# Kkuntal990/video-to-video-diffusion

Measured on AMD Instinct MI355X. Metric: ddim_steps_per_sec, higher is better.
Workload: dtype bf16; 1 GPU; DDIM-50 step (U-Net eval + update) on latent [1, 8, 48, 128, 128] = 8->48 slices @512x512, effective 264.66M U-Net (128x(1,2,4,4), latent 8), one volume per GPU, hipGraph-captured step; volumes_per_gpu=1, parallelism=dp1, full=False, finite_outputs=True

## Files before the change

### include/ctsi.h

```cpp
#ifndef CTSI_H
#define CTSI_H

#include <stddef.h>
#include <stdint.h>

#ifdef __cplusplus
extern "C" {
#endif

#define CTSI_OK 0
#define CTSI_ERR_INVALID (-1)
#define CTSI_ERR_UNSUPPORTED (-2)
#define CTSI_ERR_HIP (-3)

int ctsi_version(void);
int ctsi_ablation_build(void);
const char* ctsi_last_error(void);
int ctsi_device_available(void);

int ctsi_ncdhw_f32_to_ndhwc_bf16(const float* src, void* dst, int n, int c, int d, int h, int w,
                                 int c_total, int c_off, void* stream);
int ctsi_ndhwc_bf16_to_ncdhw_f32(const void* src, float* dst, int n, int c, int d, int h, int w,
                                 void* stream);
int ctsi_ncdhw_f32_to_ndhwc_f32(const float* src, float* dst, int n, int c, int d, int h, int w,
// ... 26 lines not shown
    const double* gn_sums;
    const float* gn_gamma;
    const float* gn_beta;
    int gn_groups;
    float gn_eps;
    long long gn_count;
    int gn_silu;
    void* workspace;
} ctsi_conv_out;

int ctsi_conv_plan_create(ctsi_conv_plan** plan, const ctsi_conv_desc* desc);
int ctsi_conv_plan_set_weight_cin(ctsi_conv_plan* plan, int cin_w);
int ctsi_conv_plan_set_stream_tail(ctsi_conv_plan* plan, int on);
void ctsi_conv_plan_destroy(ctsi_conv_plan* plan);
int ctsi_conv_plan_out_dims(const ctsi_conv_plan* plan, int* d_out, int* h_out, int* w_out);
size_t ctsi_conv_plan_weight_bytes(const ctsi_conv_plan* plan);
int ctsi_conv_plan_tiles(const ctsi_conv_plan* plan);
int ctsi_conv_plan_tiles_per_sample(const ctsi_conv_plan* plan);
int ctsi_conv_plan_cout_pad(const ctsi_conv_plan* plan);
size_t ctsi_conv_plan_workspace_bytes(const ctsi_conv_plan* plan);
double ctsi_conv_plan_flops(const ctsi_conv_plan* plan);
int ctsi_conv_plan_config(const ctsi_conv_plan* plan, int* bm, int* bn, int* mode);
int ctsi_conv_plan_form(const ctsi_conv_plan* plan, int out[8]);
#define CTSI_PACK_GATHER 1
#define CTSI_PACK_GATHER_SMALL 2
#define CTSI_PACK_HALO 3
#define CTSI_PACK_K32 4
#define CTSI_PACK_HEAD 5
#define CTSI_PACK_STREAM_TAIL 6
#define CTSI_PACK_STEM 7
int ctsi_conv_plan_pack_layout(const ctsi_conv_plan* plan);
int ctsi_conv_plan_pack_weights(const ctsi_conv_plan* plan, const float* w_f32, void* packed,
                                void* stream);
int ctsi_conv_fwd(const ctsi_conv_plan* plan, const void* x1, const void* x2, const void* packed_w,
                  const float* bias, const ctsi_conv_out* out, void* stream);

int ctsi_gn_colsum(const void* x_bf16, float* colsum, int n, int c, int d, int h, int w,
                   int* tiles_per_sample, void* stream);
int ctsi_gn_colsum_tiles(int d, int h, int w);
int ctsi_gn_finalize(const float* colsum, double* sums, int n, int c, int c_pad, int groups,
                     int tiles_per_sample, int nclass, int accumulate, void* stream);
int ctsi_gn_apply(const void* x_bf16, void* y_bf16, const double* sums, const float* gamma,
                  const float* beta, int n, int c, int d, int h, int w, int d_stat, int groups, float eps,
                  int silu_pre, const float* tbias, int tbias_stride, const int* step_ptr,
                  const void* residual_bf16, int silu_post, void* stream);

// ... 201 lines not shown
```

### video-to-video-diffusion_amd/csrc/conv3_halo_k32.hip

```cpp
#include "conv3_halo_common.h"
#include <stdlib.h>
#include <type_traits>

template <int NJ, bool DIRECT>
__device__ __forceinline__ int hk_col(int j, int r16) { return DIRECT ? r16 * NJ + j : j * 16 + r16; }

template <int TD_, int TH_, int TW_ = 32, int BN_ = 128, int UPS_ = 2>
struct HkCfg {
    static constexpr int TD = TD_, TH = TH_, TW = TW_, UPS = UPS_;
    static constexpr int HD = TD + 2, HH = TH + 2, HW = TW + 2;
    static constexpr int HV = HD * HH * HW;
    static constexpr int HALO_INSTR = (HV + 31) / 32;
    static constexpr int HALO_BYTES = HALO_INSTR * 1024;
    static constexpr int BM = TD * TH * TW;
    static constexpr int BN = BN_;
    static constexpr int NJ = BN / 16;
    static constexpr int TAP_BYTES = BN * 32;
    static constexpr int STEP_TAPS = 2 * UPS;
    static constexpr int WSLOT_BYTES = STEP_TAPS * TAP_BYTES;
    static constexpr int NWS = 4;
    static constexpr int NWAVE = 8;
    static constexpr int MA = BM / 128;
    static constexpr int NTH = 64 * NWAVE;
    static constexpr int NPIECE = (HALO_INSTR + NWAVE - 1) / NWAVE;
// ... 35 lines not shown
#if defined(__HIP_DEVICE_COMPILE__)
    using Cfg = HkCfg<TD_, TH_, TW_, BN_, UPS_>;
    constexpr int UPS = Cfg::UPS, NJ = Cfg::NJ, NJH = Cfg::NJ / 2, STEP_TAPS = Cfg::STEP_TAPS;
    constexpr int TAPS = (TR || DS) ? 12 : 27;
    static_assert(!(TR && DS), "one form at a time");
    constexpr int MA = Cfg::MA;
    constexpr int TH = Cfg::TH, TW = Cfg::TW, HH = Cfg::HH, HW = Cfg::HW, HV = Cfg::HV;
    constexpr int HALO_INSTR = Cfg::HALO_INSTR, HALO_BYTES = Cfg::HALO_BYTES, BM = Cfg::BM, BN = Cfg::BN;
    constexpr int TAP_BYTES = Cfg::TAP_BYTES, WSLOT_BYTES = Cfg::WSLOT_BYTES, NWS = Cfg::NWS, NWAVE = Cfg::NWAVE;
    constexpr int NTH = Cfg::NTH, NPIECE = Cfg::NPIECE, OFF_W = Cfg::OFF_W, OFF_ROW = Cfg::OFF_ROW, OFF_CS = Cfg::OFF_CS;
    constexpr int BNP = Cfg::BNP;
    extern __shared__ __attribute__((aligned(16))) char smem[];
    long long* s_rowoff = reinterpret_cast<long long*>(smem + OFF_ROW);
    float* s_cs = reinterpret_cast<float*>(smem + OFF_CS);

    const int tid = threadIdx.x;
    const int lane = tid & 63;
    const int wave = __builtin_amdgcn_readfirstlane(tid >> 6);

    HK_STAMP(0);
    if ((CTSI_DBG(p.dbg, 4096)) && tid == 0 && blockIdx.x < HK_NSTAMP)
        g_hk_stamps[blockIdx.x][7] = ((unsigned long long)__builtin_amdgcn_s_getreg((31 << 11) | (0 << 6) | 20) << 32) |
                                     (unsigned)__builtin_amdgcn_s_getreg((31 << 11) | (0 << 6) | 4);
    int bid = xcd_remap_h(blockIdx.x, gridDim.x);
    const int khalf = SK ? (bid & 1) : 0;
    if (SK) bid >>= 1;
    int mt, nt, cls = 0;
    if (TR) {
        const int ns = 4 * p.ntiles_n;
        const int G = (p.n_major > 0 && p.n_major < ns && ns % p.n_major == 0) ? p.n_major : ns;
        const int per_g = p.mtiles * G;
        const int sg = bid / per_g;
        const int rem = bid - sg * per_g;
        mt = rem / G;
        const int sib = sg * G + (rem - mt * G);
        cls = sib / p.ntiles_n;
        nt = sib - cls * p.ntiles_n;
    } else {
        h3_decode_tile(bid, p.mtiles, p.ntiles_n, p.n_major, &mt, &nt);
    }
    const int py = cls >> 1, px = cls & 1;
    const int n0 = nt * BN;
    const int nchunks = SK ? p.nchunks / 2 : p.nchunks;
    const int cbase = khalf * nchunks;
    const int nb = mt / p.tps;
    int r0 = mt - nb * p.tps;
    int tD, tH, tW;
    if (p.tile_order == 1) {
        tH = r0 / (p.tilesD * p.tilesW);
        r0 -= tH * p.tilesD * p.tilesW;
        tD = r0 / p.tilesW;
        tW = r0 - tD * p.tilesW;
    } else if (p.tile_order == 2 && (p.tilesW & 3) == 0 && (p.tilesH & 7) == 0) {
        tD = r0 / (p.tilesH * p.tilesW);
        r0 -= tD * p.tilesH * p.tilesW;
        const int st = r0 >> 5, in = r0 & 31, spr = p.tilesW >> 2;
        tW = (st % spr) * 4 + (in & 3);
        tH = (st / spr) * 8 + (in >> 2);
    } else {
        tD = r0 / (p.tilesH * p.tilesW);
        r0 -= tD * p.tilesH * p.tilesW;
        tH = r0 / p.tilesW;
        tW = r0 - tH * p.tilesW;
    }
    const int d0 = tD * Cfg::TD, h0 = tH * TH, w0 = tW * TW;

// ... 227 lines not shown
                hfree = ((TAPS * hc - 1) >> 1) / UPS;
                ++hc;
            }
        }
        if (s + NWS - 1 < S && !(CTSI_DBG(p.dbg, 2))) {
            issue_weights(s + NWS - 1);
            n_w = 2;
        }
        n_prev = urgent ? n_w : n_w + n_halo;
        __builtin_amdgcn_sched_barrier(0);
    };
#define HK_UNIT(FAc, FAn, BADDR, UU, BADDR_N, UU_N, AADDR_N, MID)                                              \
    {                                                                                                          \
        if (!(CTSI_DBG(p.dbg, 128))) HK_LOAD_B(fbh, NJH, BADDR, UU);    \
        HK_LOAD_A(FAn, 0, AADDR_N);                                                                            \
        HK_MFMA(FAc, fbl, 0);                                                                                  \
        HK_SCHED();                                                                                            \
        MID;                                                                                                   \
        HK_LOAD_A(FAn, 2, AADDR_N);                                                                            \
        HK_LOAD_B(fbl, 0, BADDR_N, UU_N);                                                                      \
        HK_MFMA(FAc, fbh, NJH);                                                                                \
        HK_SCHED();                                                                                            \
    }
    for (int s = 0; s < S; ++s) {
        const int baddr = b_lane + (s % NWS) * WSLOT_BYTES;
        const int baddr_n = b_lane + ((s + 1) % NWS) * WSLOT_BYTES;
        const int q0 = STEP_TAPS * s;
        int an[UPS];
#pragma unroll
        for (int k = 0; k < UPS; ++k) {
            const int oa = tap_off(q0 + 2 * k + 2), ob = tap_off(q0 + 2 * k + 3);
            an[k] = a_lane + (tap1 ? ob : oa);
        }
        HK_UNIT(fa0, fa1, baddr, 0, baddr, 1, an[0], );
        if constexpr (UPS == 4) {
            HK_UNIT(fa1, fa0, baddr, 1, baddr, 2, an[1], );
            HK_UNIT(fa0, fa1, baddr, 2, baddr, 3, an[2], );
        }
        hk_wait_vm(n_prev);
        if (!(CTSI_DBG(p.dbg, 64))) __builtin_amdgcn_s_barrier();
        __builtin_amdgcn_sched_barrier(0);
        HK_UNIT(fa1, fa0, baddr, UPS - 1, baddr_n, 0, an[UPS - 1], if (wave < 4 || (CTSI_DBG(p.dbg, 16))) issue_group(s));
        if (wave >= 4 && !(CTSI_DBG(p.dbg, 16))) issue_group(s);
    }
#undef HK_UNIT
#undef HK_LOAD_A
#undef HK_LOAD_B
#undef HK_MFMA
#undef HK_SCHED
    HK_STAMP(2);
    asm volatile("s_waitcnt vmcnt(0) lgkmcnt(0)" ::: "memory");
    if (!(DIRECT && !SK) || (p.dbg_epi_barrier != 0)) __syncthreads();
    HK_STAMP(3);

    if (CTSI_DBG(p.dbg, 8)) return;
    if (SK) {
        const int tile = mt * p.ntiles_n + nt;
        constexpr int NREG = MA * NJ * 4;
        float* wsl = p.sk_ws + (size_t)tile * NREG * NTH + tid;
        int* s_role = reinterpret_cast<int*>(s_cs);
        if (tid == 0) {
            const int tk = __hip_atomic_fetch_add(p.sk_sync + 2 * tile, 1, __ATOMIC_RELAXED, __HIP_MEMORY_SCOPE_AGENT);
            if (tk >= 2) {
                atomicAdd(&g_hk_device_error[0], 1u);
                g_hk_device_error[1] = (unsigned)tile;
            }
            *s_role = tk & 1;
        }
        __syncthreads();
        const int role = *s_role;
        __syncthreads();
        if (role == 0) {
#pragma unroll
            for (int i = 0; i < MA; ++i)
#pragma unroll
                for (int j = 0; j < NJ; ++j)
#pragma unroll
                    for (int q = 0; q < 4; ++q)
                        __hip_atomic_store(wsl + (size_t)((i * NJ + j) * 4 + q) * NTH, acc[i][j][q], __ATOMIC_RELAXED,
                                           __HIP_MEMORY_SCOPE_AGENT);
            asm volatile("s_waitcnt vmcnt(0)" ::: "memory");
            __syncthreads();
            if (tid == 0) __hip_atomic_store(p.sk_sync + 2 * tile + 1, 1, __ATOMIC_RELAXED, __HIP_MEMORY_SCOPE_AGENT);
            return;
        }
        if (tid == 0) {
            int spins = 0;
            while (__hip_atomic_load(p.sk_sync + 2 * tile + 1, __ATOMIC_RELAXED, __HIP_MEMORY_SCOPE_AGENT) == 0 && spins < (1 << 22)) {
                __builtin_amdgcn_s_sleep(4);
                ++spins;
            }
            if (spins >= (1 << 22)) {
                atomicAdd(&g_hk_device_error[0], 1u);
                g_hk_device_error[1] = (unsigned)tile;
            } else {
                __hip_atomic_store(p.sk_sync + 2 * tile, 0, __ATOMIC_RELAXED, __HIP_MEMORY_SCOPE_AGENT);
                __hip_atomic_store(p.sk_sync + 2 * tile + 1, 0, __ATOMIC_RELAXED, __HIP_MEMORY_SCOPE_AGENT);
            }
        }
        __syncthreads();
#pragma unroll
        for (int i = 0; i < MA; ++i)
#pragma unroll
            for (int j = 0; j < NJ; ++j)
#pragma unroll
                for (int q = 0; q < 4; ++q)
                    acc[i][j][q] += __hip_atomic_load(wsl + (size_t)((i * NJ + j) * 4 + q) * NTH, __ATOMIC_RELAXED,
                                                      __HIP_MEMORY_SCOPE_AGENT);
    }
    bf16_t* s_tile = reinterpret_cast<bf16_t*>(smem);
    const bool want_sums = p.colsum != nullptr;
    unsigned vbits = 0;
#pragma unroll
    for (int i = 0; i < MA; ++i)
#pragma unroll
        for (int q = 0; q < 4; ++q)
            vbits |= (unsigned)(s_rowoff[wave * 16 * MA + 16 * i + (VPERM ? 4 * q + kg : 4 * kg + q)] >= 0) << (4 * i + q);
    auto tile_out = [&](auto masked_tag, auto sums_tag) {
        constexpr bool MASKED = decltype(masked_tag)::value, SUMS = decltype(sums_tag)::value;
#pragma unroll
        for (int j = 0; j < NJ; ++j) {
            const int col = hk_col<NJ, DIRECT>(j, r16);
            float s1 = 0.0f, s2 = 0.0f;
// ... 196 lines not shown
    return CTSI_OK;
}

extern "C" int ctsi_conv3_halo_k32_direct(int tile, int ksplit, int ds) {
#ifdef HK_STAGED_EPILOGUE
    return 0;
#else
    const bool t512 = tile == 0 || tile == 2, narrow = tile == 6 || tile == 7;
    return (t512 || narrow || (tile == 5 && ksplit == 2 && !ds)) ? 1 : 0;
#endif
}

template <int TD, int TH, int TW, int BN, int UPS, bool TR, bool SK = false, bool DS = false>
static void hk_launch(const Conv3HaloParams* hp, hipStream_t stream) {
    using Cfg = HkCfg<TD, TH, TW, BN, UPS>;
#ifdef HK_STAGED_EPILOGUE
    constexpr bool DIRECT = false;
#else
    constexpr bool DIRECT = TD * TH * TW == 512 || TW == 24 || TW == 12 || (SK && !DS);
#endif
    auto k = conv3_halo_k32_kernel<TD, TH, TW, BN, UPS, TR, SK, DS, DIRECT>;
    static CtsiPerDeviceOnce attr_once;
    if (attr_once.first()) hipFuncSetAttribute((const void*)k, hipFuncAttributeMaxDynamicSharedMemorySize, 160 * 1024);
    hipLaunchKernelGGL(k, dim3((TR ? 4 : 1) * (SK ? 2 : 1) * hp->mtiles * hp->ntiles_n), dim3(Cfg::NTH), Cfg::LDS_BYTES, stream,
                       *hp);
}

extern "C" size_t ctsi_conv3_halo_k32_splitk_bytes(int tiles) {
    const size_t sync = ((size_t)tiles * 8 + 255) / 256 * 256;
    return sync + (size_t)tiles * (4 * 8 * 4) * 512 * sizeof(float);
}

extern "C" int ctsi_conv3_halo_k32_launch(const Conv3HaloParams* hp, int tile ,
                                          int bn, void* stream) {
    CTSI_CHECK_ARG(bn == 128 && (tile == 0 || tile == 2 || tile == 3 || tile == 5 || tile == 6 || tile == 7),
                   "ctsi_conv3_halo_k32_launch: bad BN %d / tile %d", bn, tile);
    if (tile == 6 || tile == 7) {
        CTSI_CHECK_ARG(!(hp->ds && hp->tr) && !(hp->ksplit == 2 && (hp->ds || hp->tr)),
                       "ctsi_conv3_halo_k32_launch: tile %d has no split-K form for strided / transposed layers", tile);
        if (hp->ksplit == 2) {
            CTSI_CHECK_ARG(hp->sk_ws && hp->sk_sync && hp->nchunks % 8 == 0, "ctsi_conv3_halo_k32_launch: split-K needs its workspace");
            if (tile == 6)
                hk_launch<4, 4, 24, 128, 2, false, true>(hp, (hipStream_t)stream);
            else
                hk_launch<8, 4, 12, 128, 2, false, true>(hp, (hipStream_t)stream);
        } else if (hp->ds) {
            CTSI_CHECK_ARG(hp->Hi == 2 * hp->Ho && hp->Wi == 2 * hp->Wo && hp->C2 == 0 && hp->nchunks % 4 == 0,
                           "ctsi_conv3_halo_k32_launch: the Downsample form needs even input planes and one source");
            if (tile == 6)
                hk_launch<4, 4, 24, 128, 2, false, false, true>(hp, (hipStream_t)stream);
            else
                hk_launch<8, 4, 12, 128, 2, false, false, true>(hp, (hipStream_t)stream);
        } else if (hp->tr) {
            if (tile == 6)
                hk_launch<4, 4, 24, 128, 2, true>(hp, (hipStream_t)stream);
            else
                hk_launch<8, 4, 12, 128, 2, true>(hp, (hipStream_t)stream);
        } else if (tile == 6) {
            hk_launch<4, 4, 24, 128, 2, false>(hp, (hipStream_t)stream);
// ... 70 lines not shown
```

### video-to-video-diffusion_amd/csrc/conv_mfma.hip

```cpp
#include <type_traits>
#include "conv3_halo_common.h"
#include "conv_plan.h"
#include <string.h>
#include <stdlib.h>
#include <math.h>


__device__ __attribute__((aligned(256))) uint32_t g_ctsi_zero_page[64];

struct ConvKParams {
    const bf16_t* x1;
    const bf16_t* x2;
    const bf16_t* w;
    const float* bias;
    void* y;
    float* colsum;
    int C1, C2, Cin;
    int Di, Hi, Wi;
    int Dr, Hr, Wr;
    int sH, sW;
    int lTH, lTW;
    int linear;
    int tilesD, tilesH, tilesW, tps, mtiles;
    int ntiles_n;
// ... 797 lines not shown
            if (p->d.transposed && !nm) h.n_major = 4;
        }
        {
            h.dbg = ctsi_debug_flags();
            h.nchunks = ctsi_debug_ksteps(h.nchunks);
        }
        {
            const char* to = getenv("CTSI_CONV_TILE_ORDER");
            h.tile_order = to ? atoi(to) : 2;
            const char* eb = getenv("CTSI_CONV_EPI_BARRIER");
            h.dbg_epi_barrier = eb ? atoi(eb) : 0;
        }
        if (family == CONV_HEAD) {
            if (p->head2 && o->colsum == nullptr)
                return ctsi_conv3_head2_launch(&h, p->d.n, (const char*)packed_w + head1_bytes(p), o->mode, o->act, o->sn, o->sc, o->sd,
                                               o->sh, o->sw, stream);
            return ctsi_conv3_head_launch(&h, p->d.cout <= 8 ? 8 : 16, o->mode, o->act, o->sn, o->sc, o->sd, o->sh, o->sw, stream);
        }
        h.tr = p->d.transposed;
        if (family == CONV_K32 && p->ksplit == 2) {
            CTSI_CHECK_ARG(o->workspace, "ctsi_conv_fwd: this plan needs ctsi_conv_out.workspace (ctsi_conv_plan_workspace_bytes)");
            const int tiles = p->mtiles * p->ntiles_n;
            h.ksplit = 2;
            h.sk_sync = (int*)o->workspace;
            h.sk_ws = (float*)((char*)o->workspace + ((size_t)tiles * 8 + 255) / 256 * 256);
        }
        if (family == CONV_K32) return ctsi_conv3_halo_k32_launch(&h, p->form->code, p->BN, stream);
        return ctsi_conv3_halo_launch(&h, p->form->code, stream);
    }
    CTSI_CHECK_ARG(!p->form, "ctsi_conv_fwd: the 3x3x3 halo-tile plan supports bf16 NDHWC output without activation");
    ConvKParams k;
    memset(&k, 0, sizeof(k));
    k.x1 = (const bf16_t*)x1;
    k.x2 = (const bf16_t*)(x2 ? x2 : x1);
    k.w = (const bf16_t*)packed_w;
    k.bias = bias;
    k.y = o->y;
    k.colsum = o->colsum;
    k.C1 = p->d.c1; k.C2 = p->d.c2; k.Cin = p->Cin;
    k.Di = p->d.di; k.Hi = p->d.hi; k.Wi = p->d.wi;
    k.Dr = p->Dr; k.Hr = p->Hr; k.Wr = p->Wr;
    k.sH = p->sH; k.sW = p->sW;
    k.lTH = p->lTH; k.lTW = p->lTW;
    k.linear = p->linear;
    k.tilesD = p->tilesD; k.tilesH = p->tilesH; k.tilesW = p->tilesW; k.tps = p->tps; k.mtiles = p->mtiles;
    k.ntiles_n = p->ntiles_n;
// ... 46 lines not shown
```

### video-to-video-diffusion_amd/csrc/conv_plan.h

```cpp
#pragma once
#include "ctsi_internal.h"

#define CTSI_MAX_TAPS 48
#define CTSI_BK 64

enum ConvFamily {
    CONV_GATHER,
    CONV_HALO32,
    CONV_K32,
    CONV_HEAD,
};

struct ConvForm {
    ConvFamily family;
    int mode;
    int td, th, tw;
    int bn;
    int code;
    double eff;
    const char* name;
};

struct ctsi_conv_plan {
    ctsi_conv_desc d;
    int Cin, CinW;
    int Do, Ho, Wo;
    int Dr, Hr, Wr, sH, sW, uH, uW;
    int nclass, T;
    int small, lcpt, kc_per_tap, ksteps, Ktot;
    int BM, BN, CoutPad, ntiles_n;
    int lTH, lTW, TD, TH, TW, tilesD, tilesH, tilesW, tps, mtiles;
    int linear;
    int tapk[CTSI_MAX_TAPS];
    int tapdelta[CTSI_MAX_TAPS];
    int8_t od[CTSI_MAX_TAPS], oh[CTSI_MAX_TAPS], ow[CTSI_MAX_TAPS];
    int NA, NB, NC;
    int ad[4][4], bh[4][4], cw[4][4];
    int8_t pH[4], pW[4];
    int tap_margin[4], ad_min[4];
    int fast, dshift;
    const ConvForm* form;
    int gsplit;
    int ds;
    int head2;
    int ksplit;
    int stem;
    int stream1;
    double flops;
};

static inline ConvFamily conv_family(const ctsi_conv_plan* p) { return p->form ? p->form->family : CONV_GATHER; }
static inline int conv_k32_image(const ctsi_conv_plan* p) { return p->ds ? 2 : p->d.transposed; }
static inline int conv_k32_direct(const ctsi_conv_plan* p) { return ctsi_conv3_halo_k32_direct(p->form->code, p->ksplit, p->ds); }
static inline size_t head1_bytes(const ctsi_conv_plan* p) {
    return ((size_t)p->Cin * 27 * (p->d.cout <= 8 ? 8 : 16) * 2 + 1024 + 255) / 256 * 256;
}
```

### video-to-video-diffusion_amd/csrc/conv_plan.hip

```cpp
#include "conv_plan.h"
#include <string.h>
#include <stdlib.h>

static const double EFF_HALO32 = 1.0, EFF_HALO32_192 = 0.95, EFF_K32_512 = 1.15, EFF_K32_384 = 1.1, EFF_K32_NARROW = 1.07;
static const double EFF_PICK_W16 = 0.85, EFF_PICK_512 = 1.1, EFF_PICK_512_W16 = 1.0;
static const double EFF_ST_512 = 1.0, EFF_ST_384 = 0.96;
static const double EFF_GATHER_STANDIN = 0.6;

enum FormId { H32_4x2x32, H32_4x4x16, H32_3x4x16, K32_4x4x32, K32_4x8x16, K32_3x4x32, K32_3x8x16, K32_4x4x24, K32_8x4x12, HEAD_4x2x16,
              N_FORMS };
static const ConvForm FORMS[N_FORMS] = {
    {CONV_HALO32, 4, 4, 2, 32, 128, 1, EFF_HALO32, "halo32 4x2x32"},
    {CONV_HALO32, 4, 4, 4, 16, 128, 3, EFF_HALO32, "halo32 4x4x16"},
    {CONV_HALO32, 4, 3, 4, 16, 128, 4, EFF_HALO32_192, "halo32 3x4x16"},
    {CONV_K32, 9, 4, 4, 32, 128, 0, EFF_K32_512, "k32 4x4x32"},
    {CONV_K32, 9, 4, 8, 16, 128, 2, EFF_K32_512, "k32 4x8x16"},
    {CONV_K32, 9, 3, 4, 32, 128, 3, EFF_K32_384, "k32 3x4x32"},
    {CONV_K32, 9, 3, 8, 16, 128, 5, EFF_K32_384, "k32 3x8x16"},
    {CONV_K32, 9, 4, 4, 24, 128, 6, EFF_K32_NARROW, "k32 4x4x24"},
    {CONV_K32, 9, 8, 4, 12, 128, 7, EFF_K32_NARROW, "k32 8x4x12"},
    {CONV_HEAD, 8, 4, 2, 16, 16, 0, 1.0, "head 4x2x16"},
};
static int form_voxels(const ConvForm& f) { return f.td * f.th * f.tw; }
static const ConvForm* k32_sized(const ConvForm* f, bool v384) {
    return &FORMS[f->tw == 16 ? (v384 ? K32_3x8x16 : K32_4x8x16) : (v384 ? K32_3x4x32 : K32_4x4x32)];
}

enum Tri { UNSET = -1, OFF = 0, ON = 1 };
enum SplitK { SK_UNSET, SK_OFF, SK_ON, SK_PLAIN, SK_512 };
struct PlanEnv {
    bool no_halo3, force_halo3, no_c16, no_head3, no_head2, no_fast;
    Tri m512, m512w16, k32_384, k32t, k32d, narrow, narrow_sk, linear;
    int halo_tile;
    int h32w16;
    SplitK splitk;
    int sk384_min, sk512_min;
    bool has_gsplit; int gsplit;
    int tile_bm, tile_bn;
};
static Tri env_tri(const char* name) {
    const char* e = getenv(name);
    return e && !strcmp(e, "0") ? OFF : e && !strcmp(e, "1") ? ON : UNSET;
}
static int env_int(const char* name, int unset) {
    const char* e = getenv(name);
    return e ? atoi(e) : unset;
}
static PlanEnv read_plan_env() {
    PlanEnv e;
    e.no_halo3 = getenv("CTSI_CONV_NO_HALO3") != nullptr;
    e.force_halo3 = getenv("CTSI_CONV_FORCE_HALO3") != nullptr;
    e.no_c16 = getenv("CTSI_CONV_NO_C16") != nullptr;
    e.no_head3 = getenv("CTSI_CONV_NO_HEAD3") != nullptr;
    e.no_head2 = getenv("CTSI_CONV_NO_HEAD2") != nullptr;
    e.no_fast = getenv("CTSI_CONV_NO_FAST") != nullptr;
    e.m512 = env_tri("CTSI_CONV_M512");
    e.m512w16 = env_tri("CTSI_CONV_M512W16");
    e.k32_384 = env_tri("CTSI_CONV_K32_384");
    e.k32t = env_tri("CTSI_CONV_K32T");
    e.k32d = env_tri("CTSI_CONV_K32D");
    e.narrow = env_tri("CTSI_CONV_K32_NARROW");
    e.narrow_sk = env_tri("CTSI_CONV_K32_NARROW_SK");
    e.linear = env_tri("CTSI_CONV_LINEAR");
    const char* hv = getenv("CTSI_CONV_HALO_TILE");
    e.halo_tile = hv && !strcmp(hv, "16") ? 16 : hv && !strcmp(hv, "32") ? 32 : 0;
    const char* hw = getenv("CTSI_CONV_H32W16");
    e.h32w16 = hw && !strcmp(hw, "1") ? 1 : hw && !strcmp(hw, "2") ? 2 : 0;
    const char* sk = getenv("CTSI_CONV_K32_SPLITK");
    e.splitk = !sk ? SK_UNSET : !strcmp(sk, "0") ? SK_OFF : !strcmp(sk, "1") ? SK_ON : !strcmp(sk, "plain") ? SK_PLAIN
               : !strcmp(sk, "512") ? SK_512 : SK_UNSET;
    e.sk384_min = env_int("CTSI_CONV_K32_SK384_MIN", 256);
    e.sk512_min = env_int("CTSI_CONV_K32_SK512_MIN", 512);
    const char* gs = getenv("CTSI_CONV_GSPLIT");
    e.has_gsplit = gs != nullptr;
    e.gsplit = gs ? atoi(gs) : 0;
    const char* tile = getenv("CTSI_CONV_TILE");
    e.tile_bm = tile && !strcmp(tile, "128x128") ? 128 : tile && (!strcmp(tile, "256x128") || !strcmp(tile, "256x256")) ? 256 : 0;
    e.tile_bn = tile && !strcmp(tile, "256x256") ? 256 : 128;
    return e;
}

static double cu_rounds(long long b) { return (double)(((b + 255) / 256) * 256); }
static double cu_fill(long long b) { return (double)b / cu_rounds(b); }
static long long plan_rows(const ctsi_conv_plan* p) { return (long long)p->Dr * p->Hr * p->Wr; }
static long long padded_rows(const ctsi_conv_plan* p, const ConvForm& f) {
// ... 230 lines not shown
    p->ds = ds;
    if (e.m512w16 != UNSET) p->form = &FORMS[e.m512w16 == ON ? K32_4x8x16 : K32_4x4x32];
    if (e.k32_384 != UNSET) p->form = k32_sized(p->form, e.k32_384 == ON);
    if (ds) {
        const long long t5 = fit(p, FORMS[K32_3x8x16], 1, 1, 1.0).blocks;
        bool use_sk = p->Cin % 32 == 0 && p->Cin >= 256 && bf.blocks <= 160 && 2 * t5 <= 512;
        if (e.splitk == SK_OFF) use_sk = false;
        if (e.splitk == SK_ON && p->Cin % 32 == 0) use_sk = true;
        if (use_sk) {
            p->form = &FORMS[K32_3x8x16];
            p->ksplit = 2;
        }
    }
}

static void choose_head_form(ctsi_conv_plan* p, const PlanEnv& e) {
    const ctsi_conv_desc& d = p->d;
    if (p->form || !is_k3(d) || p->small || d.c2 != 0 || d.c1 % 32 != 0 || d.cout > 16 || !halo_fits(p) || e.no_head3) return;
    if (!covers_70(p, HEAD_4x2x16) && !e.force_halo3) return;
    p->form = &FORMS[HEAD_4x2x16];
    p->head2 = ctsi_conv3_head2_supported(p->Cin, d.cout) && !e.no_head2;
}

static void finish_tiles(ctsi_conv_plan* p) {
    p->CoutPad = ceil_div(p->d.cout, p->BN) * p->BN;
    p->ntiles_n = p->CoutPad / p->BN;
    p->lTH = ilog2(p->TH); p->lTW = ilog2(p->TW);
    p->tilesD = ceil_div(p->Dr, p->TD);
    p->tilesH = ceil_div(p->Hr, p->TH);
    p->tilesW = ceil_div(p->Wr, p->TW);
    p->tps = p->tilesD * p->tilesH * p->tilesW;
    p->mtiles = p->d.n * p->tps;
}

static void choose_linear_rows(ctsi_conv_plan* p, const PlanEnv& e) {
    const long long rows = plan_rows(p), boxed = (long long)p->tps * p->BM;
    if (!((boxed * 100 > rows * 115 && e.linear != OFF) || e.linear == ON)) return;
    p->linear = 1;
    p->tps = (int)((rows + p->BM - 1) / p->BM);
    p->mtiles = p->d.n * p->tps;
    p->TD = (int)(p->BM / ((long long)p->Hr * p->Wr)) + 2;
}

static void choose_gather_split(ctsi_conv_plan* p, const PlanEnv& e) {
    if (p->small || p->BM != 128 || p->BN != 128) return;
    const long long blocks = (long long)p->nclass * p->mtiles * p->ntiles_n;
// ... 22 lines not shown
                   "ctsi_conv_plan_create: bad kernel/stride");
    ctsi_conv_plan* p = (ctsi_conv_plan*)calloc(1, sizeof(ctsi_conv_plan));
    CTSI_CHECK_ARG(p, "ctsi_conv_plan_create: out of host memory");
    p->d = d;
    const int rc = plan_geometry(p);
    if (rc != CTSI_OK) {
        free(p);
        return rc;
    }
    const PlanEnv e = read_plan_env();
    plan_k_walk(p);
    choose_gather_tile(p, e);
    if (is_k3(d)) choose_k3_form(p, e);
    else choose_k32_strided_form(p, e);
    choose_head_form(p, e);
    if (p->form) {
        p->BM = form_voxels(*p->form);
        p->BN = p->form->bn;
        p->TD = p->form->td; p->TH = p->form->th; p->TW = p->form->tw;
    } else {
        choose_box_tile(p);
    }
    finish_tiles(p);
    if (!p->form) choose_linear_rows(p, e);
    {
        const int cmax = d.c1 > d.c2 ? d.c1 : d.c2;
        const double extent = ((double)(p->TD + 4) * d.hi * d.wi + 2.0 * d.wi + 8) * cmax * 2.0;
        p->fast = !p->small && d.c1 % 64 == 0 && d.c2 % 64 == 0 && extent < 2.0e9 && !e.no_fast;
    }
    if (!p->form) choose_gather_split(p, e);
    *out = p;
    return CTSI_OK;
}

extern "C" void ctsi_conv_plan_destroy(ctsi_conv_plan* plan) { free(plan); }

extern "C" int ctsi_conv_plan_out_dims(const ctsi_conv_plan* p, int* d, int* h, int* w) {
    CTSI_CHECK_ARG(p, "ctsi_conv_plan_out_dims: null plan");
    if (d) *d = p->Do;
    if (h) *h = p->Ho;
    if (w) *w = p->Wo;
    return CTSI_OK;
}
extern "C" size_t ctsi_conv_plan_weight_bytes(const ctsi_conv_plan* p) {
    if (!p) return 0;
    if (p->stem) return ctsi_conv3_stem_weight_bytes(p->CoutPad);
    if (p->stream1) return (size_t)p->d.cout * p->Cin * 2;
    switch (conv_family(p)) {
    case CONV_HEAD:
        return head1_bytes(p) + (ctsi_conv3_head2_supported(p->Cin, p->d.cout) ? ctsi_conv3_head2_weight_bytes(p->d.cout) : 0);
    case CONV_K32: return ctsi_conv3_halo_k32_weight_bytes(p->Cin, p->CoutPad, p->BN, conv_k32_image(p));
    case CONV_HALO32: return (size_t)p->Cin * 27 * p->CoutPad * 2;
    default: return (size_t)p->nclass * p->CoutPad * p->Ktot * 2;
    }
}
extern "C" int ctsi_conv_plan_tiles(const ctsi_conv_plan* p) { return p ? p->nclass * p->mtiles : 0; }
extern "C" int ctsi_conv_plan_tiles_per_sample(const ctsi_conv_plan* p) { return p ? p->tps : 0; }
extern "C" int ctsi_conv_plan_cout_pad(const ctsi_conv_plan* p) { return p ? p->CoutPad : 0; }
extern "C" double ctsi_conv_plan_flops(const ctsi_conv_plan* p) { return p ? p->flops : 0.0; }
extern "C" size_t ctsi_conv_plan_workspace_bytes(const ctsi_conv_plan* p) {
    if (p && !p->form && p->gsplit >= 2) {
        const size_t tiles = (size_t)p->nclass * p->mtiles * p->ntiles_n;
        return (tiles * 4 + 255) / 256 * 256 + tiles * p->gsplit * (size_t)(128 * 128) * sizeof(float);
    }
    if (!p || p->ksplit != 2) return 0;
    return ctsi_conv3_halo_k32_splitk_bytes(p->mtiles * p->ntiles_n);
}
extern "C" int ctsi_conv_plan_config(const ctsi_conv_plan* p, int* bm, int* bn, int* mode) {
    CTSI_CHECK_ARG(p, "ctsi_conv_plan_config: null plan");
    if (bm) *bm = p->stream1 ? 16 : p->BM;
    if (bn) *bn = p->stream1 ? p->stream1 * 16 : p->BN;
    if (mode) *mode = p->stem ? 11 : p->stream1 ? 10 : (p->form ? p->form->mode : (p->small ? 1 : (p->fast ? 2 : 0)));
    return CTSI_OK;
}

extern "C" int ctsi_conv_plan_form(const ctsi_conv_plan* p, int out[8]) {
    CTSI_CHECK_ARG(p && out, "ctsi_conv_plan_form: null argument");
    memset(out, 0, 8 * sizeof(int));
    out[0] = p->TD; out[1] = p->TH; out[2] = p->TW;
    if (!p->stem && !p->stream1) out[3] = conv_family(p) == CONV_K32 ? p->ksplit : (p->form ? 0 : p->gsplit);
    out[4] = (p->linear ? 1 : 0) | (p->fast ? 2 : 0) | (p->head2 ? 4 : 0) | (p->ds ? 8 : 0);
    return CTSI_OK;
}

extern "C" int ctsi_conv_plan_pack_layout(const ctsi_conv_plan* p) {
    if (!p) return 0;
    if (p->stem) return CTSI_PACK_STEM;
    if (p->stream1) return CTSI_PACK_STREAM_TAIL | (p->stream1 << 8);
    switch (conv_family(p)) {
    case CONV_K32: return CTSI_PACK_K32 | (conv_k32_image(p) << 4) | (conv_k32_direct(p) << 6) | ((p->BN / 16) << 8);
// ... 33 lines not shown
```

### video-to-video-diffusion_amd/csrc/ctsi_internal.h

```cpp
#pragma once
#include <hip/hip_runtime.h>
#include <stdint.h>
#include <stdio.h>
#include <stdarg.h>
#include "../../include/ctsi.h"

typedef uint16_t bf16_t;

typedef __attribute__((ext_vector_type(8))) short bf16x8;
typedef __attribute__((ext_vector_type(4))) float f32x4;
typedef __attribute__((ext_vector_type(16))) float f32x16;

void ctsi_set_error(const char* fmt, ...);

#define CTSI_CHECK_ARG(cond, ...)            \
    do {                                     \
        if (!(cond)) {                       \
            ctsi_set_error(__VA_ARGS__);     \
            return CTSI_ERR_INVALID;         \
        }                                    \
    } while (0)

struct CtsiPerDeviceOnce {
    bool done[64] = {};
// ... 83 lines not shown
    const float* bias;
    void* y;
    float* colsum;
    int C1, C2;
    int Di, Hi, Wi;
    int Do, Ho, Wo;
    int dshift;
    int tilesD, tilesH, tilesW, tps, mtiles, ntiles_n;
    int nchunks;
    int Cout, CoutPad;
    int cout_stride, c_off;
    int n_major;
    int dbg;
    const double* nin_sums;
    const float* nin_gamma;
    const float* nin_beta;
    const float* nin_tbias;
    const int* nin_step_ptr;
    int nin_tb_stride, nin_groups, nin_silu, nin_n_total;
    int nin_pad_lo, nin_pad_hi;
    float nin_eps;
    double nin_count;
    int ksplit;
    float* sk_ws;
    int* sk_sync;
    int tr;
    int ds;
    int tile_order;
    int nt_store;
    int dbg_epi_barrier;
};

extern "C" int ctsi_conv3_halo_pack(const float* w, void* packed, int cout, int cout_pad, int cin, int cin_w,
                                    void* stream);
extern "C" int ctsi_conv3_halo_launch(const Conv3HaloParams* hp, int wide, void* stream);
extern "C" int ctsi_conv3_head_launch(const Conv3HaloParams* hp, int rows, int out_mode, int act, long long sn, long long sc,
                                      long long sd, long long sh, long long sw, void* stream);
extern "C" int ctsi_conv3_head2_supported(int cin, int cout);
extern "C" size_t ctsi_conv3_head2_weight_bytes(int cout);
extern "C" int ctsi_conv3_head2_pack(const float* w, void* packed, int cout, int cin, int cin_w, void* stream);
extern "C" int ctsi_conv3_head2_launch(const Conv3HaloParams* hp, int n, const void* packed, int out_mode, int act, long long sn,
                                       long long sc, long long sd, long long sh, long long sw, void* stream);
struct StemParams {
    const bf16_t* x;
    const bf16_t* w;
    const float* bias;
// ... 41 lines not shown
```

### video-to-video-diffusion_amd/lib.py

```python
from __future__ import annotations

import ctypes as C
import os
import subprocess
from pathlib import Path

_PKG_DIR = Path(__file__).resolve().parent
LIB_PATH = _PKG_DIR / "libctsi.so"
CSRC_DIR = _PKG_DIR / "csrc"
HEADER_PATH = _PKG_DIR.parent / "include" / "ctsi.h"


class CtsiError(RuntimeError):
    """Raised when libctsi is unavailable or one of its entry points reports an error."""


class ConvDesc(C.Structure):
    _fields_ = [
        ("transposed", C.c_int),
        ("kd", C.c_int), ("kh", C.c_int), ("kw", C.c_int),
        ("sh", C.c_int), ("sw", C.c_int),
        ("pd", C.c_int), ("ph", C.c_int), ("pw", C.c_int),
        ("n", C.c_int), ("c1", C.c_int), ("c2", C.c_int),
        ("cout", C.c_int),
# ... 37 lines not shown
SIGNATURES = {
    "ctsi_version": (_i, [], False),
    "ctsi_ablation_build": (_i, [], False),
    "ctsi_last_error": (C.c_char_p, [], False),
    "ctsi_device_available": (_i, [], False),
    "ctsi_ncdhw_f32_to_ndhwc_bf16": (_i, [_vp, _vp, _i, _i, _i, _i, _i, _i, _i, _vp], True),
    "ctsi_ndhwc_bf16_to_ncdhw_f32": (_i, [_vp, _vp, _i, _i, _i, _i, _i, _vp], True),
    "ctsi_ncdhw_f32_to_ndhwc_f32": (_i, [_vp, _vp, _i, _i, _i, _i, _i, _vp], True),
    "ctsi_ndhwc_f32_to_ncdhw_f32": (_i, [_vp, _vp, _i, _i, _i, _i, _i, _vp], True),
    "ctsi_conv_plan_create": (_i, [C.POINTER(_vp), C.POINTER(ConvDesc)], True),
    "ctsi_conv_plan_set_weight_cin": (_i, [_vp, _i], True),
    "ctsi_conv_plan_set_stream_tail": (_i, [_vp, _i], True),
    "ctsi_conv_plan_destroy": (None, [_vp], False),
    "ctsi_conv_plan_out_dims": (_i, [_vp, _ip, _ip, _ip], True),
    "ctsi_conv_plan_weight_bytes": (_sz, [_vp], False),
    "ctsi_conv_plan_workspace_bytes": (_sz, [_vp], False),
    "ctsi_conv_plan_tiles": (_i, [_vp], False),
    "ctsi_conv_plan_tiles_per_sample": (_i, [_vp], False),
    "ctsi_conv_plan_cout_pad": (_i, [_vp], False),
    "ctsi_conv_plan_flops": (C.c_double, [_vp], False),
    "ctsi_conv_plan_config": (_i, [_vp, _ip, _ip, _ip], True),
    "ctsi_conv_plan_pack_layout": (_i, [_vp], False),
    "ctsi_conv_plan_form": (_i, [_vp, _ip], True),
    "ctsi_conv_plan_pack_weights": (_i, [_vp, _vp, _vp, _vp], True),
    "ctsi_conv_fwd": (_i, [_vp, _vp, _vp, _vp, _vp, C.POINTER(ConvOut), _vp], True),
    "ctsi_gn_colsum": (_i, [_vp, _vp, _i, _i, _i, _i, _i, _ip, _vp], True),
    "ctsi_gn_colsum_tiles": (_i, [_i, _i, _i], False),
    "ctsi_gn_finalize": (_i, [_vp, _vp, _i, _i, _i, _i, _i, _i, _i, _vp], True),
    "ctsi_gn_apply": (_i, [_vp, _vp, _vp, _vp, _vp, _i, _i, _i, _i, _i, _i, _i, _f, _i, _vp, _i, _vp, _vp,
                           _i, _vp], True),
    "ctsi_attn_depthsum": (_i, [_vp, _vp, _vp, _i, _i, _i, _i, _i, _vp], True),
    "ctsi_attn_depthsum_tiles": (_i, [_i, _i, _i], False),
    "ctsi_attn_normsum": (_i, [_vp, _vp, _vp, _vp, _vp, _i, _i, _i, _i, _i, _i, _f, _vp], True),
    "ctsi_attn_pv_supported": (_i, [_i, _i], False),
    "ctsi_attn_pv": (_i, [_vp, _vp, _vp, _vp, _vp, _vp, _vp, _i, _i, _i, _i, _i, _i, _f, _vp], True),
    "ctsi_attn_broadcast_add": (_i, [_vp, _vp, _vp, _i, _vp, _i, _i, _i, _i, _i, _vp], True),
    "ctsi_attn_softmax_rowsum": (_i, [_vp, _vp, _i, _i, _i, _i, _i, _i, _vp], True),
    "ctsi_time_embed_fwd": (_i, [_vp, _i, _i, _i, _vp, _vp, _vp, _vp, _vp, _vp, _i, _vp, _vp, _vp], True),
    "ctsi_time_embed_fwd_tf": (_i, [_vp, _i, _i, _i, _vp, _vp, _vp, _vp, _vp, _vp, _i, _vp, _vp, _vp], True),
    "ctsi_trilinear_depth_fwd": (_i, [_vp, _vp, _i, _i, _i, _i, _i, _i, _i, _i, _vp, _vp], True),
    "ctsi_ddim_step": (_i, [_vp, _vp, _vp, _vp, _i, _i, _vp, _vp, _i, _i, _i, _i, _i, _vp, _vp], True),
    "ctsi_ddpm_step": (_i, [_vp, _vp, _vp, _vp, _i, _i, _vp, _vp, _i, _i, _i, _i, _i, _vp], True),
    "ctsi_ddpm_posterior": (_i, [_vp, _vp, _vp, _vp, _vp, _vp, _i, _ll, _i, _vp], True),
    "ctsi_step_advance": (_i, [_vp, _vp], True),
    "ctsi_nan_to_num_f32": (_i, [_vp, _ll, _vp], True),
    "ctsi_count_nonfinite_f32": (_i, [_vp, _ll, _i, _vp, _vp], True),
# ... 141 lines not shown
```

Before: 39.75 steps/s.

## Add hybrid split-K scheduling that splits only the tail wave of k32 conv tiles

For split-K k32 halo convolutions whose per-XCD tile count leaves a partial final wave, most tiles now run unsplit and only the tail remainder uses split-K. The launch grid shrinks accordingly, and blocks are remapped per XCD so unsplit and split units interleave. The aim is to drop the split-K workspace reduction overhead on most tiles while keeping load balance on the last wave. It adds complexity to tile decoding and a mid-loop accumulator store path whose correctness depends on the XCD layout assumptions.

After: 39.69 steps/s. Within noise of the previous version (-0.2%).

```diff
diff --git a/include/ctsi.h b/include/ctsi.h
--- a/include/ctsi.h
+++ b/include/ctsi.h
@@ -72,6 +72,7 @@
 double ctsi_conv_plan_flops(const ctsi_conv_plan* plan);
 int ctsi_conv_plan_config(const ctsi_conv_plan* plan, int* bm, int* bn, int* mode);
 int ctsi_conv_plan_form(const ctsi_conv_plan* plan, int out[8]);
+int ctsi_conv_plan_splitk_full_units(const ctsi_conv_plan* plan);
 #define CTSI_PACK_GATHER 1
 #define CTSI_PACK_GATHER_SMALL 2
 #define CTSI_PACK_HALO 3
diff --git a/video-to-video-diffusion_amd/csrc/conv3_halo_k32.hip b/video-to-video-diffusion_amd/csrc/conv3_halo_k32.hip
--- a/video-to-video-diffusion_amd/csrc/conv3_halo_k32.hip
+++ b/video-to-video-diffusion_amd/csrc/conv3_halo_k32.hip
@@ -81,9 +81,23 @@
     if ((CTSI_DBG(p.dbg, 4096)) && tid == 0 && blockIdx.x < HK_NSTAMP)
         g_hk_stamps[blockIdx.x][7] = ((unsigned long long)__builtin_amdgcn_s_getreg((31 << 11) | (0 << 6) | 20) << 32) |
                                      (unsigned)__builtin_amdgcn_s_getreg((31 << 11) | (0 << 6) | 4);
-    int bid = xcd_remap_h(blockIdx.x, gridDim.x);
-    const int khalf = SK ? (bid & 1) : 0;
-    if (SK) bid >>= 1;
+    constexpr bool HYBRID = SK && !TR && !DS;
+    int bid, khalf = 0;
+    bool split_rt = true;
+    if (HYBRID && p.sk_full_x > 0) {
+        const int u = (p.mtiles * p.ntiles_n) >> 3, f = p.sk_full_x;
+        const int xcd = blockIdx.x & 7, l = blockIdx.x >> 3;
+        split_rt = l >= f;
+        bid = xcd * u + (split_rt ? f + ((l - f) >> 1) : l);
+        khalf = split_rt ? (l - f) & 1 : 0;
+    } else {
+        bid = xcd_remap_h(blockIdx.x, gridDim.x);
+        if (SK) {
+            khalf = bid & 1;
+            bid >>= 1;
+        }
+    }
+    const bool split = HYBRID ? split_rt : SK;
     int mt, nt, cls = 0;
     if (TR) {
         const int ns = 4 * p.ntiles_n;
@@ -100,7 +114,7 @@
     }
     const int py = cls >> 1, px = cls & 1;
     const int n0 = nt * BN;
-    const int nchunks = SK ? p.nchunks / 2 : p.nchunks;
+    const int nchunks = split ? p.nchunks / 2 : p.nchunks;
     const int cbase = khalf * nchunks;
     const int nb = mt / p.tps;
     int r0 = mt - nb * p.tps;
@@ -374,7 +388,29 @@
         HK_MFMA(FAc, fbh, NJH);                                                                                \
         HK_SCHED();                                                                                            \
     }
-    for (int s = 0; s < S; ++s) {
+    const int nseg = (HYBRID && !split) ? 2 : 1, S_seg = S / nseg;
+    constexpr int NREG = MA * NJ * 4;
+    auto ws_slot = [&]() -> float* {
+        int t = tid;
+        asm volatile("" : "+v"(t));
+        return p.sk_ws + (size_t)(mt * p.ntiles_n + nt) * NREG * NTH + t;
+    };
+    for (int seg = 0; seg < nseg; ++seg) {
+    if (HYBRID && seg > 0) {
+        float* wsl = ws_slot();
+#pragma unroll
+        for (int i = 0; i < MA; ++i)
+#pragma unroll
+            for (int j = 0; j < NJ; ++j)
+#pragma unroll
+                for (int q = 0; q < 4; ++q) {
+                    __hip_atomic_store(wsl + (size_t)((i * NJ + j) * 4 + q) * NTH, acc[i][j][q], __ATOMIC_RELAXED,
+                                       __HIP_MEMORY_SCOPE_AGENT);
+                    acc[i][j][q] = 0.0f;
+                }
+        __builtin_amdgcn_sched_barrier(0);
+    }
+    for (int s = seg * S_seg; s < (seg + 1 == nseg ? S : (seg + 1) * S_seg); ++s) {
         const int baddr = b_lane + (s % NWS) * WSLOT_BYTES;
         const int baddr_n = b_lane + ((s + 1) % NWS) * WSLOT_BYTES;
         const int q0 = STEP_TAPS * s;
@@ -394,6 +430,7 @@
         __builtin_amdgcn_sched_barrier(0);
         HK_UNIT(fa1, fa0, baddr, UPS - 1, baddr_n, 0, an[UPS - 1], if (wave < 4 || (CTSI_DBG(p.dbg, 16))) issue_group(s));
         if (wave >= 4 && !(CTSI_DBG(p.dbg, 16))) issue_group(s);
+    }
     }
 #undef HK_UNIT
 #undef HK_LOAD_A
@@ -402,14 +439,14 @@
 #undef HK_SCHED
     HK_STAMP(2);
     asm volatile("s_waitcnt vmcnt(0) lgkmcnt(0)" ::: "memory");
-    if (!(DIRECT && !SK) || (p.dbg_epi_barrier != 0)) __syncthreads();
+    if (!(DIRECT && !split) || (p.dbg_epi_barrier != 0)) __syncthreads();
     HK_STAMP(3);
 
     if (CTSI_DBG(p.dbg, 8)) return;
     if (SK) {
+      float* wsl = ws_slot();
+      if (split) {
         const int tile = mt * p.ntiles_n + nt;
-        constexpr int NREG = MA * NJ * 4;
-        float* wsl = p.sk_ws + (size_t)tile * NREG * NTH + tid;
         int* s_role = reinterpret_cast<int*>(s_cs);
         if (tid == 0) {
             const int tk = __hip_atomic_fetch_add(p.sk_sync + 2 * tile, 1, __ATOMIC_RELAXED, __HIP_MEMORY_SCOPE_AGENT);
@@ -451,6 +488,7 @@
             }
         }
         __syncthreads();
+      }
 #pragma unroll
         for (int i = 0; i < MA; ++i)
 #pragma unroll
@@ -693,7 +731,8 @@
     auto k = conv3_halo_k32_kernel<TD, TH, TW, BN, UPS, TR, SK, DS, DIRECT>;
     static CtsiPerDeviceOnce attr_once;
     if (attr_once.first()) hipFuncSetAttribute((const void*)k, hipFuncAttributeMaxDynamicSharedMemorySize, 160 * 1024);
-    hipLaunchKernelGGL(k, dim3((TR ? 4 : 1) * (SK ? 2 : 1) * hp->mtiles * hp->ntiles_n), dim3(Cfg::NTH), Cfg::LDS_BYTES, stream,
+    const int units = hp->mtiles * hp->ntiles_n;
+    hipLaunchKernelGGL(k, dim3((TR ? 4 : 1) * (SK ? 2 * units - 8 * hp->sk_full_x : units)), dim3(Cfg::NTH), Cfg::LDS_BYTES, stream,
                        *hp);
 }
 
@@ -706,6 +745,9 @@
                                           int bn, void* stream) {
     CTSI_CHECK_ARG(bn == 128 && (tile == 0 || tile == 2 || tile == 3 || tile == 5 || tile == 6 || tile == 7),
                    "ctsi_conv3_halo_k32_launch: bad BN %d / tile %d", bn, tile);
+    CTSI_CHECK_ARG(hp->sk_full_x == 0 || (hp->ksplit == 2 && !hp->tr && !hp->ds && (hp->mtiles * hp->ntiles_n) % 8 == 0 &&
+                                          hp->sk_full_x > 0 && hp->sk_full_x <= hp->mtiles * hp->ntiles_n / 8),
+                   "ctsi_conv3_halo_k32_launch: %d unsplit units per XCD do not fit this split-K launch", hp->sk_full_x);
     if (tile == 6 || tile == 7) {
         CTSI_CHECK_ARG(!(hp->ds && hp->tr) && !(hp->ksplit == 2 && (hp->ds || hp->tr)),
                        "ctsi_conv3_halo_k32_launch: tile %d has no split-K form for strided / transposed layers", tile);
diff --git a/video-to-video-diffusion_amd/csrc/conv_mfma.hip b/video-to-video-diffusion_amd/csrc/conv_mfma.hip
--- a/video-to-video-diffusion_amd/csrc/conv_mfma.hip
+++ b/video-to-video-diffusion_amd/csrc/conv_mfma.hip
@@ -843,6 +843,7 @@
             CTSI_CHECK_ARG(o->workspace, "ctsi_conv_fwd: this plan needs ctsi_conv_out.workspace (ctsi_conv_plan_workspace_bytes)");
             const int tiles = p->mtiles * p->ntiles_n;
             h.ksplit = 2;
+            h.sk_full_x = p->sk_full / 8;
             h.sk_sync = (int*)o->workspace;
             h.sk_ws = (float*)((char*)o->workspace + ((size_t)tiles * 8 + 255) / 256 * 256);
         }
diff --git a/video-to-video-diffusion_amd/csrc/conv_plan.h b/video-to-video-diffusion_amd/csrc/conv_plan.h
--- a/video-to-video-diffusion_amd/csrc/conv_plan.h
+++ b/video-to-video-diffusion_amd/csrc/conv_plan.h
@@ -44,6 +44,7 @@
     int ds;
     int head2;
     int ksplit;
+    int sk_full;
     int stem;
     int stream1;
     double flops;
diff --git a/video-to-video-diffusion_amd/csrc/conv_plan.hip b/video-to-video-diffusion_amd/csrc/conv_plan.hip
--- a/video-to-video-diffusion_amd/csrc/conv_plan.hip
+++ b/video-to-video-diffusion_amd/csrc/conv_plan.hip
@@ -30,7 +30,7 @@
 enum SplitK { SK_UNSET, SK_OFF, SK_ON, SK_PLAIN, SK_512 };
 struct PlanEnv {
     bool no_halo3, force_halo3, no_c16, no_head3, no_head2, no_fast;
-    Tri m512, m512w16, k32_384, k32t, k32d, narrow, narrow_sk, linear;
+    Tri m512, m512w16, k32_384, k32t, k32d, narrow, narrow_sk, linear, sk_hybrid;
     int halo_tile;
     int h32w16;
     SplitK splitk;
@@ -61,6 +61,7 @@
     e.k32d = env_tri("CTSI_CONV_K32D");
     e.narrow = env_tri("CTSI_CONV_K32_NARROW");
     e.narrow_sk = env_tri("CTSI_CONV_K32_NARROW_SK");
+    e.sk_hybrid = env_tri("CTSI_CONV_K32_SK_HYBRID");
     e.linear = env_tri("CTSI_CONV_LINEAR");
     const char* hv = getenv("CTSI_CONV_HALO_TILE");
     e.halo_tile = hv && !strcmp(hv, "16") ? 16 : hv && !strcmp(hv, "32") ? 32 : 0;
@@ -337,6 +338,14 @@
     p->head2 = ctsi_conv3_head2_supported(p->Cin, d.cout) && !e.no_head2;
 }
 
+static int splitk_full_units(const ctsi_conv_plan* p, const PlanEnv& e) {
+    if (p->ksplit != 2 || conv_family(p) != CONV_K32 || p->ds || p->d.transposed || e.sk_hybrid == OFF) return 0;
+    const long long U = (long long)p->mtiles * p->ntiles_n;
+    if (U % 8 != 0) return 0;
+    const long long u = U / 8, rem = u % 32;
+    return (u >= 32 && rem > 0 && rem <= 16) ? (int)(8 * (u - rem)) : 0;
+}
+
 static void finish_tiles(ctsi_conv_plan* p) {
     p->CoutPad = ceil_div(p->d.cout, p->BN) * p->BN;
     p->ntiles_n = p->CoutPad / p->BN;
@@ -405,6 +414,7 @@
         choose_box_tile(p);
     }
     finish_tiles(p);
+    p->sk_full = splitk_full_units(p, e);
     if (!p->form) choose_linear_rows(p, e);
     {
         const int cmax = d.c1 > d.c2 ? d.c1 : d.c2;
@@ -449,6 +459,7 @@
     if (!p || p->ksplit != 2) return 0;
     return ctsi_conv3_halo_k32_splitk_bytes(p->mtiles * p->ntiles_n);
 }
+extern "C" int ctsi_conv_plan_splitk_full_units(const ctsi_conv_plan* p) { return p && !p->stem && !p->stream1 ? p->sk_full : 0; }
 extern "C" int ctsi_conv_plan_config(const ctsi_conv_plan* p, int* bm, int* bn, int* mode) {
     CTSI_CHECK_ARG(p, "ctsi_conv_plan_config: null plan");
     if (bm) *bm = p->stream1 ? 16 : p->BM;
diff --git a/video-to-video-diffusion_amd/csrc/ctsi_internal.h b/video-to-video-diffusion_amd/csrc/ctsi_internal.h
--- a/video-to-video-diffusion_amd/csrc/ctsi_internal.h
+++ b/video-to-video-diffusion_amd/csrc/ctsi_internal.h
@@ -129,6 +129,7 @@
     float nin_eps;
     double nin_count;
     int ksplit;
+    int sk_full_x;
     float* sk_ws;
     int* sk_sync;
     int tr;
diff --git a/video-to-video-diffusion_amd/lib.py b/video-to-video-diffusion_amd/lib.py
--- a/video-to-video-diffusion_amd/lib.py
+++ b/video-to-video-diffusion_amd/lib.py
@@ -83,6 +83,7 @@
     "ctsi_conv_plan_config": (_i, [_vp, _ip, _ip, _ip], True),
     "ctsi_conv_plan_pack_layout": (_i, [_vp], False),
     "ctsi_conv_plan_form": (_i, [_vp, _ip], True),
+    "ctsi_conv_plan_splitk_full_units": (_i, [_vp], False),
     "ctsi_conv_plan_pack_weights": (_i, [_vp, _vp, _vp, _vp], True),
     "ctsi_conv_fwd": (_i, [_vp, _vp, _vp, _vp, _vp, C.POINTER(ConvOut), _vp], True),
     "ctsi_gn_colsum": (_i, [_vp, _vp, _i, _i, _i, _i, _i, _ip, _vp], True),
```
